# hellobertrand/zxc

Hardware: AMD Instinct MI355X
Metric: seekable decode GB/s (level 3, 64 KiB independent blocks, HBM-resident in/out) (higher is better)
Workload: dtype u8

## Files before the change

### zxc_amd/csrc/zxc_decode_kernel.hip

```cpp
#include "zxc_experiments.h"
#include <hip/hip_runtime.h>
#include <stdint.h>

#include "zxc_kernels.h"
#include "zxc_wave.h"

typedef unsigned __int128 u128;

#include "zxc_lds.h"

#define RING_BYTES 4096u
#define RING_MASK (RING_BYTES - 1u)
#define RING_WORDS (RING_BYTES / 4u)
#define REDIRECT_PASSES 2
#define SPARSE_MAX 8
#define TILE_MAX 3584u
#define LIT_MED 128u
#define MATCH_MED 128u
#define BYTEWISE_MAX 32u

#define E_DST_TOO_SMALL (-2)
#define E_SRC_TOO_SMALL (-3)
#define E_BAD_HEADER (-6)
#define E_BAD_CHECKSUM (-7)
// ... 1133 lines not shown
    }
#ifdef EXP_TIMES
    __builtin_amdgcn_s_waitcnt(0);
    {
        const uint64_t t_end = wall_clock64();
        rc = (int)((((uint32_t)(t_start >> 5) & 0xFFFFu) << 16) | (uint32_t)(((t_end - t_start) >> 5) & 0xFFFFu));
    }
#endif
    if (lane == 0) status[b] = rc == ZXC_DEV_DEFER ? ZXC_DEV_E_INTERNAL : rc;
}

extern "C" __global__ void __launch_bounds__(64, LEAN_WAVES_PER_SIMD)
zxc_decode_blocks_lean_kernel(const uint8_t* __restrict__ comp, const zxc_dev_job_t* __restrict__ jobs, uint32_t n_jobs,
                              uint8_t* __restrict__ out, int32_t* __restrict__ status, uint32_t block_size,
                              const uint32_t* __restrict__ order, uint32_t cap_override, uint32_t trailer_bytes,
                              const zxc_dev_pre_t* __restrict__ pre, const uint8_t* __restrict__ rscratch) {
    __shared__ LeanLds L;
    if (blockIdx.x >= n_jobs) return;
    const uint32_t b = order ? uni(order[blockIdx.x]) : blockIdx.x;
    const uint32_t cls = uni(pre[b].cls);
    if (cls != ZXC_DEV_CLS_LEAN && cls != ZXC_DEV_CLS_LEAN_RLE) return;
    const uint8_t* rle_slot = cls == ZXC_DEV_CLS_LEAN_RLE ? rscratch + 16ull * uni(pre[b].lit_off) : nullptr;
    const int rle_rc = cls == ZXC_DEV_CLS_LEAN_RLE ? (int)(int16_t)uni((uint32_t)(uint16_t)pre[b].rc_lit) : 0;
    lean_one_block<false>(comp, jobs, out, status, block_size, cap_override, trailer_bytes, b, nullptr, nullptr, L, threadIdx.x, rle_slot, rle_rc);
}

extern "C" __global__ void __launch_bounds__(64)
zxc_rle_expand_kernel(const uint8_t* __restrict__ comp, const zxc_dev_job_t* __restrict__ jobs, zxc_dev_pre_t* __restrict__ pre,
                      uint8_t* __restrict__ rscratch, const uint32_t* __restrict__ hdr, const uint32_t* __restrict__ entries_last) {
    const int lane = threadIdx.x;
    const uint32_t n = uni(hdr[0]);
    for (uint32_t i = blockIdx.x; i < n; i += gridDim.x) {
        const uint32_t b = uni(*(entries_last - i));
        const uint8_t* src = comp + jobs[b].comp_off;
        const uint32_t n_lit = uni(ld32(src + 12));
        int rc = 0;
        if (n_lit != 0u) rc = rle_expand(src + 8 + 16, uni(ld32(src + 20)), rscratch + 16ull * uni(pre[b].lit_off) + 16u, n_lit, lane);
        if (lane == 0) pre[b].rc_lit = (int16_t)rc;
    }
}

extern "C" __global__ void __launch_bounds__(64, LEAN_WAVES_PER_SIMD)
zxc_decode_blocks_lean_pre_kernel(const uint8_t* __restrict__ comp, const zxc_dev_job_t* __restrict__ jobs, uint8_t* __restrict__ out,
                                  int32_t* __restrict__ status, uint32_t block_size, uint32_t cap_override, uint32_t trailer_bytes,
                                  const zxc_dev_pre_t* __restrict__ pre, const uint8_t* __restrict__ pscratch,
                                  const uint32_t* __restrict__ hdr, const uint32_t* __restrict__ entries) {
    __shared__ LeanLds L;
    if (blockIdx.x >= uni(hdr[0])) return;
    lean_one_block<true>(comp, jobs, out, status, block_size, cap_override, trailer_bytes, uni(entries[blockIdx.x]), pre, pscratch, L, threadIdx.x, nullptr, 0);
}

extern "C" __global__ void __launch_bounds__(64)
zxc_block_checksum_kernel(const uint8_t* __restrict__ comp, const zxc_dev_job_t* __restrict__ jobs, uint32_t n_jobs,
                          const uint32_t* __restrict__ order, uint8_t* __restrict__ ck_bad) {
    const int lane = threadIdx.x;
    const uint32_t slot = blockIdx.x * 9u + (uint32_t)lane / 7u;
    const bool in = lane < 63 && slot < n_jobs;
    const uint32_t b = in ? (order ? order[slot] : slot) : 0u;
    const uint8_t* src = comp + jobs[b].comp_off;
    const uint32_t src_sz = in ? jobs[b].comp_size : 0u;
    uint32_t comp_sz = 0;
    bool on = false;
    if (src_sz >= 8u) {
        comp_sz = ld32(src + 3);
        on = (uint64_t)8u + comp_sz + 4u <= src_sz;
    }
    const uint32_t h = group_checksum32(src + 8, on ? comp_sz : 0u, lane, on);
    if (on && lane % 7 == 0) ck_bad[b] = h != ld32(src + 8 + comp_sz) ? 1u : 0u;
    else if (in && !on && lane % 7 == 0) ck_bad[b] = 0u;
}
extern "C" __global__ void __launch_bounds__(256)
zxc_checksum_merge_kernel(const uint8_t* __restrict__ ck_bad, int32_t* __restrict__ status, uint32_t n_jobs) {
    const uint32_t i = blockIdx.x * 256u + threadIdx.x;
    if (i < n_jobs && ck_bad[i]) status[i] = E_BAD_CHECKSUM;
}

__device__ __forceinline__ uint32_t order_bucket(const uint8_t* __restrict__ comp, const zxc_dev_job_t& j, uint32_t block_size) {
    uint32_t cost = 0;
    if (j.comp_size >= 8u + 12u) {
        const uint8_t* h = comp + j.comp_off;
        const uint32_t type = ld8(h);
        if (type == 1u || type == 2u) {
            const uint32_t n_seq = ld32(h + 8), n_lit = ld32(h + 12), enc_lit = ld8(h + 16), enc_tok = ld8(h + 17);
            cost = n_seq + (enc_tok == 2u ? n_seq : 0u) + (enc_lit == 1u ? n_lit >> 4 : 0u) + (enc_lit >= 2u ? n_lit >> 2 : 0u);
        }
    }
    const uint64_t q = (uint64_t)cost * 320u / block_size;
    return 63u - (q > 63u ? 63u : (uint32_t)q);
}

extern "C" __global__ void __launch_bounds__(256)
zxc_order_hist_kernel(const uint8_t* __restrict__ comp, const zxc_dev_job_t* __restrict__ jobs, uint32_t n_jobs,
                      uint32_t block_size, uint32_t* __restrict__ hist) {
    __shared__ uint32_t cnt[64];
    if (threadIdx.x < 64u) cnt[threadIdx.x] = 0;
    __syncthreads();
    const uint32_t i = blockIdx.x * 256u + threadIdx.x;
    if (i < n_jobs) atomicAdd(cnt + order_bucket(comp, jobs[i], block_size), 1u);
    __syncthreads();
    if (threadIdx.x < 64u && cnt[threadIdx.x]) atomicAdd(hist + threadIdx.x, cnt[threadIdx.x]);
}

extern "C" __global__ void __launch_bounds__(256)
zxc_order_scatter_kernel(const uint8_t* __restrict__ comp, const zxc_dev_job_t* __restrict__ jobs, uint32_t n_jobs,
                         uint32_t block_size, uint32_t* __restrict__ hist, uint32_t* __restrict__ order,
                         uint32_t* __restrict__ list, uint32_t trailer_bytes, zxc_dev_pre_t* __restrict__ pre,
                         uint32_t* __restrict__ ctl, uint32_t* __restrict__ pre_entries, zxc_dev_sec_t* __restrict__ secs,
                         uint32_t pscratch_cap16, uint32_t cap, uint32_t rscratch_cap16) {
    __shared__ uint32_t cnt[64], base[64];
    __shared__ uint32_t wg_cnt[8], wg_base[8];
    __shared__ uint32_t wg_fit, wg_rle_fit;
    if (threadIdx.x < 64u) cnt[threadIdx.x] = 0;
    if (threadIdx.x < 8u) wg_cnt[threadIdx.x] = 0;
    __syncthreads();
    const uint32_t i = blockIdx.x * 256u + threadIdx.x;
    uint32_t bk = 0, rank = 0;
    if (i < n_jobs) {
        bk = order_bucket(comp, jobs[i], block_size);
        rank = atomicAdd(cnt + bk, 1u);
    }
    __syncthreads();
    if (threadIdx.x < 64u) {
        uint32_t s = 0;
        for (uint32_t k = 0; k < threadIdx.x; k++) s += hist[k];
        base[threadIdx.x] = cnt[threadIdx.x] ? s + atomicAdd(hist + 64u + threadIdx.x, cnt[threadIdx.x]) : 0u;
    }
    __syncthreads();
    if (i < n_jobs) order[base[bk] + rank] = i;
    if (!list) return;
    BlockClass c = {ZXC_DEV_CLS_LEAN, 0, 0, 3, 3, 0, 0, 0, 0, 0, 0};
    uint32_t my_off = 0, my_pre = 0, my_full = 0, my_lit = 0, my_tok = 0;
    if (i < n_jobs) {
        c = classify_block(comp + jobs[i].comp_off, jobs[i].comp_size, trailer_bytes, block_size, cap);
        if (c.cls == ZXC_DEV_CLS_PRE) {
            my_off = atomicAdd(wg_cnt + 0, c.lit16 + c.tok16);
            my_pre = atomicAdd(wg_cnt + 1, 1u);
            if (c.lit_cls < 3u) my_lit = atomicAdd(wg_cnt + 3u + c.lit_cls, 1u);
            if (c.tok_cls < 3u) my_tok = atomicAdd(wg_cnt + 3u + c.tok_cls, 1u);
        } else if (c.cls == ZXC_DEV_CLS_FULL) {
            my_full = atomicAdd(wg_cnt + 2, 1u);
        } else if (c.cls == ZXC_DEV_CLS_LEAN_RLE) {
            my_off = atomicAdd(wg_cnt + 6, c.lit16);
            my_pre = atomicAdd(wg_cnt + 7, 1u);
        }
    }
    __syncthreads();
    if (threadIdx.x == 0) {
        bool rfit = rscratch_cap16 != 0u;
        wg_base[6] = 0;
        if (wg_cnt[7]) {
            atomicAdd(ctl + ZXC_DEV_CTL_RLE_WANTED, wg_cnt[6] + 1u);
            if (wg_cnt[6]) {
                uint32_t old = __hip_atomic_load(ctl + ZXC_DEV_CTL_RLE_CURSOR, __ATOMIC_RELAXED, __HIP_MEMORY_SCOPE_AGENT);
                for (;;) {
                    if (old > rscratch_cap16) { rfit = false; break; }
                    const uint32_t seen = atomicCAS(ctl + ZXC_DEV_CTL_RLE_CURSOR, old, old + wg_cnt[6]);
                    if (seen == old) { rfit = (uint64_t)old + wg_cnt[6] <= rscratch_cap16; break; }
                    old = seen;
                }
                wg_base[6] = old;
            }
            if (!rfit) wg_cnt[2] += wg_cnt[7];
            else wg_base[7] = atomicAdd(ctl + ZXC_DEV_CTL_RLE_LIST, wg_cnt[7]);
        }
        wg_rle_fit = rfit ? 1u : 0u;
        bool fit = true;
        wg_base[0] = 0;
        if (wg_cnt[0]) {
            uint32_t old = __hip_atomic_load(ctl + ZXC_DEV_CTL_CURSOR, __ATOMIC_RELAXED, __HIP_MEMORY_SCOPE_AGENT);
            for (;;) {
                if (old > pscratch_cap16) { fit = false; break; }
                const uint32_t seen = atomicCAS(ctl + ZXC_DEV_CTL_CURSOR, old, old + wg_cnt[0]);
                if (seen == old) { fit = (uint64_t)old + wg_cnt[0] <= pscratch_cap16; break; }
                old = seen;
            }
            wg_base[0] = old;
        }
        wg_fit = fit ? 1u : 0u;
        if (wg_cnt[1]) atomicAdd(ctl + ZXC_DEV_CTL_WANTED, wg_cnt[1]);
        if (fit) {
            wg_base[1] = wg_cnt[1] ? atomicAdd(ctl + ZXC_DEV_CTL_PRE, wg_cnt[1]) : 0u;
            wg_base[2] = wg_cnt[2] ? atomicAdd(list, wg_cnt[2]) : 0u;
            for (uint32_t k = 0; k < 3u; k++) wg_base[3u + k] = wg_cnt[3u + k] ? atomicAdd(ctl + ZXC_DEV_CTL_SEC + 2u * k, wg_cnt[3u + k]) : 0u;
        } else {
            wg_base[2] = atomicAdd(list, wg_cnt[2] + wg_cnt[1]);
        }
    }
    __syncthreads();
    if (i >= n_jobs) return;
    uint32_t cls = c.cls;
    if (cls == ZXC_DEV_CLS_PRE && !wg_fit) {
        cls = ZXC_DEV_CLS_FULL;
        my_full = wg_cnt[2] + my_pre;
    }
    if (cls == ZXC_DEV_CLS_LEAN_RLE) {
        if (wg_rle_fit) {
            pre_entries[n_jobs - 1u - (wg_base[7] + my_pre)] = i;
            pre[i].lit_off = wg_base[6] + my_off;
            pre[i].tok_off = 0;
            pre[i].rc_lit = 0;
            pre[i].rc_tok = 0;
            pre[i].cls = cls;
            return;
        }
        cls = ZXC_DEV_CLS_FULL;
        my_full = wg_cnt[2] - wg_cnt[7] + my_pre;
    }
    const uint32_t off = wg_base[0] + my_off;
    pre[i].lit_off = off;
    pre[i].tok_off = off + c.lit16;
    pre[i].rc_lit = 0;
    pre[i].rc_tok = 0;
    pre[i].cls = cls;
    if (cls == ZXC_DEV_CLS_FULL) {
        list[2u + wg_base[2] + my_full] = base[bk] + rank;
    } else if (cls == ZXC_DEV_CLS_PRE) {
        pre_entries[wg_base[1] + my_pre] = i;
        if (c.lit_cls < 3u) {
            zxc_dev_sec_t& s = secs[(size_t)c.lit_cls * 2u * n_jobs + wg_base[3u + c.lit_cls] + my_lit];
            s.src_off = jobs[i].comp_off + c.lit_at;
            s.psize = c.lit_psize;
            s.n = c.n_lit;
            s.out_off4 = 4u * off + 4u;
            s.rc_slot = 8u * i + 4u;
        }
        if (c.tok_cls < 3u) {
            zxc_dev_sec_t& s = secs[(size_t)c.tok_cls * 2u * n_jobs + wg_base[3u + c.tok_cls] + my_tok];
            s.src_off = jobs[i].comp_off + c.tok_at;
            s.psize = c.tok_psize;
            s.n = c.n_seq;
            s.out_off4 = 4u * (off + c.lit16);
            s.rc_slot = 8u * i + 5u;
        }
    }
}
```

### zxc_amd/csrc/zxc_dev.h

```cpp
#ifndef ZXC_DEV_H
#define ZXC_DEV_H
#include "../../include/zxc_mi355x.h"

#define ZXC_DEV_E_UNSUPPORTED (-101)
#define ZXC_DEV_DEFER (-103)
#define ZXC_DEV_E_INTERNAL (-102)

typedef struct zxc_enc_job {
    uint64_t src_off;
    uint32_t len;
    uint32_t pad;
} zxc_enc_job_t;

#define ZXC_DEV_CLS_LEAN 0u
#define ZXC_DEV_CLS_FULL 1u
#define ZXC_DEV_CLS_PRE 2u
#define ZXC_DEV_CLS_LEAN_RLE 3u
typedef struct {
    uint32_t lit_off;
    uint32_t tok_off;
    int16_t rc_lit, rc_tok;
    uint32_t cls;
} zxc_dev_pre_t;
typedef struct {
    uint64_t src_off;
    uint32_t psize, n;
    uint32_t out_off4;
    uint32_t rc_slot;
    uint32_t pad[2];
} zxc_dev_sec_t;
#define ZXC_DEV_TRAILER_ELSEWHERE 0x80000000u
#define ZXC_DEV_CTL_WORDS 32u
#define ZXC_DEV_CTL_PRE 0u
#define ZXC_DEV_CTL_CURSOR 2u
#define ZXC_DEV_CTL_WANTED 3u
#define ZXC_DEV_CTL_SEC 4u
#define ZXC_DEV_CTL_RLE_CURSOR 10u
#define ZXC_DEV_CTL_RLE_WANTED 11u
#define ZXC_DEV_CTL_RLE_LIST 12u

#define ZXC_DEV_SLOT_REGION(bs) ((bs) + 64u)
#define ZXC_DEV_SLOT_STRIDE(bs) ((2u * ZXC_DEV_SLOT_REGION(bs) + (bs) / 5u + 16u + 64u + 255u) & ~255u)

typedef struct { size_t list, order, ctl, pre_ent, secs, pre, ck_bad, words; } zxc_dev_ord_layout_t;
static inline zxc_dev_ord_layout_t zxc_dev_ord_layout(uint32_t n_jobs) {
    const size_t n = n_jobs, ctl = 130u + 2u * n, pre_ent = ctl + ZXC_DEV_CTL_WORDS, secs = (pre_ent + n + 7u) & ~(size_t)7u;
    const zxc_dev_ord_layout_t l = {128u, 130u + n, ctl, pre_ent, secs, secs + 48u * n, secs + 52u * n, secs + 52u * n + (n + 3u) / 4u};
    return l;
}

enum { ZXC_DEV_PLAN_FULL, ZXC_DEV_PLAN_DICT, ZXC_DEV_PLAN_TWO_PASS, ZXC_DEV_PLAN_TWO_PASS_PRE };
#define ZXC_DEV_DBG_NO_TWO_PASS 0x40000000u
#define ZXC_DEV_DBG_NO_ORDER 0x80000000u
typedef struct {
    uint32_t kind, ordered, ck_apart, trailer_bytes;
    uint64_t pscratch_bytes, rscratch_bytes;
} zxc_dev_plan_t;
typedef struct {
    uint32_t dict, cap_override, n_jobs, max_slots, debug, verify_trailer, block_size;
    uint32_t slot, helpers, hint, hint0, hint1;
    uint32_t ck_inline, no_rle_scratch, rle_lean_max_jobs, no_pre;
    uint32_t order_failed, pscratch_failed, rscratch_failed;
} zxc_dev_plan_in_t;

static inline zxc_dev_plan_t zxc_dev_plan_choose(const zxc_dev_plan_in_t* in) {
    const uint64_t gib = (uint64_t)1 << 30, n = in->n_jobs, bs = in->block_size;
    const int two_pass = !in->dict && !in->cap_override && !(in->debug & ZXC_DEV_DBG_NO_TWO_PASS);
    const int wants_order = two_pass || (in->n_jobs > in->max_slots && !(in->debug & ZXC_DEV_DBG_NO_ORDER));
    zxc_dev_plan_t p = {in->dict ? ZXC_DEV_PLAN_DICT : ZXC_DEV_PLAN_FULL, wants_order && in->slot && !in->order_failed, 0u,
                        in->verify_trailer ? 4u : 0u, 0u, 0u};
    if (!two_pass || !p.ordered || !in->helpers) return p;
    p.kind = (!in->hint || in->hint0 != 0u) && !in->no_pre && !in->pscratch_failed ? ZXC_DEV_PLAN_TWO_PASS_PRE : ZXC_DEV_PLAN_TWO_PASS;
    if (p.kind == ZXC_DEV_PLAN_TWO_PASS_PRE) p.pscratch_bytes = n * (bs + bs / 5u + 256u) < gib ? n * (bs + bs / 5u + 256u) : gib;
    if (in->hint && n < in->rle_lean_max_jobs && in->hint1 && !in->no_rle_scratch && !in->rscratch_failed) {
        const uint64_t need = ((uint64_t)in->hint1 * 16u * 5u / 4u + 65536u) & ~(uint64_t)4095u, most = n * (bs + 96u) < gib ? n * (bs + 96u) : gib;
        p.rscratch_bytes = need < most ? need : most;
    }
    p.ck_apart = p.kind == ZXC_DEV_PLAN_TWO_PASS && in->verify_trailer && !in->ck_inline;
    if (p.ck_apart) p.trailer_bytes |= ZXC_DEV_TRAILER_ELSEWHERE;
    return p;
}
#endif
```

### zxc_amd/csrc/zxc_experiments.h

```cpp
#ifndef ZXC_EXPERIMENTS_H
#define ZXC_EXPERIMENTS_H
#ifndef ZXC_EXPERIMENT
#if defined(ASM_MARKERS) || defined(EXP_ENC_CLOCKS) || defined(EXP_NO_PRE) || defined(EXP_PHASES) || defined(EXP_PIV_PROF) || defined(EXP_TIMES)
#error "an experiment switch is defined without -DZXC_EXPERIMENT: this is not the product configuration (zxc_experiments.h)"
#endif
#endif
#endif
```

### zxc_amd/csrc/zxc_hip_shim.hip

```cpp
#include "zxc_experiments.h"
#include <hip/hip_runtime.h>
#include <pthread.h>
#include <stdint.h>
#include <stdlib.h>

#include "../../include/zxc_error.h"
#include "zxc_encode_levels.h"
#include "zxc_kernels.h"

#ifdef EXP_ENC_CLOCKS
extern "C" __attribute__((visibility("default"))) int zxc_mi355x_exp_enc_clocks(unsigned long long* out8) {
    unsigned long long* d = NULL;
    if (hipMalloc((void**)&d, 64) != hipSuccess) return -1;
    hipLaunchKernelGGL(zxc_enc_clk_read_kernel, dim3(1), dim3(64), 0, 0, d);
    const hipError_t e = hipMemcpy(out8, d, 64, hipMemcpyDeviceToHost);
    (void)hipFree(d);
    return e == hipSuccess ? 0 : -1;
}
#endif

#define ZXC_MAX_DEVICES 16
#define ZXC_RLE_LEAN_MAX_JOBS 16384u
#define ZXC_ORDER_STREAMS 16
#define ZXC_POOLS 10
struct Pool { uint8_t* scratch; uint32_t* busy; uint32_t n_slots; uint32_t stride; };
struct Ord {
    void* stream; int used; uint32_t* buf; size_t buf_cap; hipStream_t aux, aux2; hipEvent_t fork, join, join2, small_done;
    uint32_t* hint; uint8_t* pscratch; size_t pscratch_cap; uint8_t* rscratch; size_t rscratch_cap;
};
static struct {
    Pool pool[ZXC_POOLS];
    int cus, wg_per_cu;
    Ord ord[ZXC_ORDER_STREAMS];
} g_dev[ZXC_MAX_DEVICES];
static pthread_mutex_t g_lock = PTHREAD_MUTEX_INITIALIZER;

#ifdef ZXC_EXPERIMENT
static uint32_t g_debug_flags = 0;
#else
#define g_debug_flags 0u
#endif

static int current_device(void) {
    int d = -1;
    if (hipGetDevice(&d) != hipSuccess || d < 0 || d >= ZXC_MAX_DEVICES) return -1;
    return d;
}

extern "C" {

#ifdef ZXC_EXPERIMENT
__attribute__((visibility("default"))) void zxc_mi355x__set_debug(uint32_t flags) { g_debug_flags = flags; }
#endif

int zxc_mi355x_device_count(void) {
    int n = 0;
    if (hipGetDeviceCount(&n) != hipSuccess) return 0;
    return n;
}

int zxc_mi355x_set_device(int device) {
    return hipSetDevice(device) == hipSuccess ? ZXC_OK : ZXC_ERROR_GPU_UNAVAILABLE;
}

int zxc_mi355x_get_device(void) {
    int d = -1;
    return hipGetDevice(&d) == hipSuccess ? d : ZXC_ERROR_GPU_UNAVAILABLE;
}

void* zxc_mi355x_malloc(size_t bytes) {
    void* p = NULL;
    if (hipMalloc(&p, bytes ? bytes : 16) != hipSuccess) return NULL;
    return p;
}

void zxc_mi355x_free(void* d_ptr) {
    if (d_ptr) (void)hipFree(d_ptr);
}

int zxc_mi355x_memcpy_h2d(void* d_dst, const void* h_src, size_t bytes) {
    if (bytes == 0) return ZXC_OK;
    return hipMemcpy(d_dst, h_src, bytes, hipMemcpyHostToDevice) == hipSuccess ? ZXC_OK : ZXC_ERROR_GPU_UNAVAILABLE;
}

int zxc_mi355x_memcpy_d2h(void* h_dst, const void* d_src, size_t bytes) {
// ... 33 lines not shown
    *ev_out = (void*)e;
    return ZXC_OK;
}
void zxc_hip_event_destroy(void* ev) { if (ev) (void)hipEventDestroy((hipEvent_t)ev); }
int zxc_hip_event_record(void* ev, void* stream) {
    return hipEventRecord((hipEvent_t)ev, (hipStream_t)stream) == hipSuccess ? ZXC_OK : ZXC_ERROR_GPU_UNAVAILABLE;
}
int zxc_hip_event_synchronize(void* ev) {
    return hipEventSynchronize((hipEvent_t)ev) == hipSuccess ? ZXC_OK : ZXC_ERROR_GPU_UNAVAILABLE;
}
void* zxc_hip_host_alloc(size_t bytes) {
    void* p = NULL;
    if (hipHostMalloc(&p, bytes ? bytes : 16, hipHostMallocDefault) != hipSuccess) return NULL;
    return p;
}
void zxc_hip_host_free(void* p) { if (p) (void)hipHostFree(p); }

extern "C" void zxc_host_release_arenas(void);
void zxc_mi355x_release_cached(void) {
    zxc_host_release_arenas();
    const int dev = current_device();
    if (dev < 0) return;
    (void)hipDeviceSynchronize();
    pthread_mutex_lock(&g_lock);
    for (int i = 0; i < ZXC_POOLS; i++) {
        auto& p = g_dev[dev].pool[i];
        if (p.scratch) (void)hipFree(p.scratch);
        if (p.busy) (void)hipFree(p.busy);
        p.scratch = NULL; p.busy = NULL; p.n_slots = 0; p.stride = 0;
    }
    for (int i = 0; i < ZXC_ORDER_STREAMS; i++) {
        auto& o = g_dev[dev].ord[i];
        if (o.buf) (void)hipFree(o.buf);
        if (o.pscratch) (void)hipFree(o.pscratch);
        if (o.rscratch) (void)hipFree(o.rscratch);
        o.buf = NULL; o.buf_cap = 0;
        o.pscratch = NULL; o.pscratch_cap = 0;
        o.rscratch = NULL; o.rscratch_cap = 0;
    }
    pthread_mutex_unlock(&g_lock);
}

int zxc_mi355x_synchronize(void* stream) {
    return hipStreamSynchronize((hipStream_t)stream) == hipSuccess ? ZXC_OK : ZXC_ERROR_GPU_UNAVAILABLE;
}

static int setup_pool(int dev, uint32_t block_size, Pool** pool_out, uint32_t* max_slots) {
    auto& d = g_dev[dev];
    if (d.cus == 0 && (hipDeviceGetAttribute(&d.cus, hipDeviceAttributeMultiprocessorCount, dev) != hipSuccess || d.cus <= 0)) d.cus = 256;
    if (d.wg_per_cu == 0 && (hipOccupancyMaxActiveBlocksPerMultiprocessor(&d.wg_per_cu, zxc_decode_blocks_kernel, 64, 0) != hipSuccess ||
                             d.wg_per_cu <= 0 || d.wg_per_cu > 32))
        d.wg_per_cu = 32;
    *max_slots = (uint32_t)d.cus * (uint32_t)d.wg_per_cu;
    Pool& pool = *(*pool_out = &d.pool[__builtin_ctz(block_size) - 12]);
    if (pool.scratch) return ZXC_OK;
    const uint32_t stride = ZXC_DEV_SLOT_STRIDE(block_size);
    uint32_t n = (uint32_t)(((size_t)1 << 30) / stride);
    if (n > *max_slots) n = *max_slots;
    if (n < 64u) n = 64u;
    uint8_t* sc = NULL;
    uint32_t* busy = NULL;
    if (hipMalloc((void**)&sc, (size_t)n * stride) != hipSuccess) return ZXC_ERROR_MEMORY;
    if (hipMalloc((void**)&busy, (size_t)n * 4u) != hipSuccess) { (void)hipFree(sc); return ZXC_ERROR_MEMORY; }
    if (hipMemset(busy, 0, (size_t)n * 4u) != hipSuccess || hipDeviceSynchronize() != hipSuccess) {
        (void)hipFree(sc), (void)hipFree(busy);
        return ZXC_ERROR_GPU_UNAVAILABLE;
    }
    pool = Pool{sc, busy, n, stride};
    return ZXC_OK;
}

static Ord* claim_slot(int dev, void* stream) {
    Ord* ord = g_dev[dev].ord;
    for (int i = 0; i < ZXC_ORDER_STREAMS; i++)
        if (ord[i].used && ord[i].stream == stream) return &ord[i];
    for (int i = 0; i < ZXC_ORDER_STREAMS; i++)
        if (!ord[i].used) {
            ord[i].used = 1, ord[i].stream = stream;
            if (ord[i].hint) { ord[i].hint[0] = 0xFFFFFFFFu; ord[i].hint[1] = 0u; }
            return &ord[i];
        }
    return NULL;
}

static void make_helpers(Ord& o) {
    if (o.aux) return;
    if (hipStreamCreateWithFlags(&o.aux, hipStreamNonBlocking) != hipSuccess) { o.aux = NULL; return; }
    const unsigned f = hipEventDisableTiming;
    if (hipStreamCreateWithFlags(&o.aux2, hipStreamNonBlocking) != hipSuccess) { (void)hipStreamDestroy(o.aux); o.aux = NULL; return; }
    if (hipEventCreateWithFlags(&o.fork, f) != hipSuccess || hipEventCreateWithFlags(&o.join, f) != hipSuccess ||
        hipEventCreateWithFlags(&o.join2, f) != hipSuccess || hipEventCreateWithFlags(&o.small_done, f) != hipSuccess) {
        (void)hipStreamDestroy(o.aux), (void)hipStreamDestroy(o.aux2);
        o.aux = NULL;
    } else if (!o.hint) {
        if (hipHostMalloc((void**)&o.hint, 64, hipHostMallocDefault) == hipSuccess) { o.hint[0] = 0xFFFFFFFFu; o.hint[1] = 0u; }
        else o.hint = NULL;
    }
}

static bool grow(void** p, size_t* cap, size_t bytes) {
    if (*cap >= bytes) return true;
    if (*p) (void)hipFree(*p);
    *cap = 0;
    if (hipMalloc(p, bytes) != hipSuccess) { *p = NULL; return false; }
    *cap = bytes;
    return true;
}

struct Launch {
    const uint8_t* comp; const zxc_dev_job_t* jobs; uint32_t n; uint8_t* out; int32_t* status; uint32_t bs, cap_override;
    zxc_dev_plan_t plan; hipStream_t s0; const Pool* pool; uint32_t max_slots, cus; Ord* o;
    uint32_t *order, *list, *ctl, *pre_entries; zxc_dev_sec_t* secs; zxc_dev_pre_t* pre;
    uint8_t *ck_bad, *pscratch, *rscratch; uint32_t pscratch_cap16, rscratch_cap16;
};

static void order_pass(const Launch& L) {
    const uint32_t g = (L.n + 255u) / 256u;
    hipLaunchKernelGGL(zxc_order_hist_kernel, dim3(g), dim3(256), 0, L.s0, L.comp, L.jobs, L.n, L.bs, L.o->buf);
    hipLaunchKernelGGL(zxc_order_scatter_kernel, dim3(g), dim3(256), 0, L.s0, L.comp, L.jobs, L.n, L.bs, L.o->buf, L.order, L.list,
                       L.plan.trailer_bytes & ~ZXC_DEV_TRAILER_ELSEWHERE, L.pre, L.ctl, L.pre_entries, L.secs, L.pscratch_cap16,
                       L.cap_override ? L.cap_override : L.bs + 2112u, L.rscratch_cap16);
    if (L.ctl && L.o->hint) {
        (void)hipMemcpyAsync(L.o->hint, L.ctl + ZXC_DEV_CTL_WANTED, 4, hipMemcpyDeviceToHost, L.s0);
        (void)hipMemcpyAsync(L.o->hint + 1, L.ctl + ZXC_DEV_CTL_RLE_WANTED, 4, hipMemcpyDeviceToHost, L.s0);
    }
}

static void launch_full(const Launch& L, hipStream_t st, uint32_t grid) {
    hipLaunchKernelGGL(zxc_decode_blocks_kernel, dim3(grid), dim3(64), 0, st, L.comp, L.jobs, L.n, L.out, L.status, L.bs, L.plan.trailer_bytes,
                       L.pool->scratch, L.pool->stride, g_debug_flags, L.pool->busy, L.pool->n_slots, L.order, L.cap_override, L.list);
}

static void launch_rle(const Launch& L, hipStream_t st) {
    if (!L.rscratch_cap16) return;
    hipLaunchKernelGGL(zxc_rle_expand_kernel, dim3(L.n < 8u * L.cus ? L.n : 8u * L.cus), dim3(64), 0, st, L.comp, L.jobs, L.pre,
                       L.rscratch, L.ctl + ZXC_DEV_CTL_RLE_LIST, L.pre_entries + L.n - 1u);
}

static bool fork_to(Ord& o, hipStream_t h) { return hipStreamWaitEvent(h, o.fork, 0) == hipSuccess; }
static int fail(Ord& o) { (void)hipStreamSynchronize(o.aux), (void)hipStreamSynchronize(o.aux2); return ZXC_ERROR_GPU_UNAVAILABLE; }
static int join(Ord& o, hipStream_t s0, bool aux, bool aux2) {
    if ((aux && (hipEventRecord(o.join, o.aux) != hipSuccess || hipStreamWaitEvent(s0, o.join, 0) != hipSuccess)) ||
        (aux2 && (hipEventRecord(o.join2, o.aux2) != hipSuccess || hipStreamWaitEvent(s0, o.join2, 0) != hipSuccess)))
        return fail(o);
    return ZXC_OK;
}

static int enqueue_two_pass(const Launch& L) {
    Ord& o = *L.o; const hipStream_t s0 = L.s0;
    const bool aux = hipEventRecord(o.fork, s0) == hipSuccess && fork_to(o, o.aux);
    launch_full(L, aux ? o.aux : s0, L.n < L.max_slots ? L.n : L.max_slots);
    const bool aux2 = L.plan.ck_apart && aux && fork_to(o, o.aux2);
    if (L.plan.ck_apart)
        hipLaunchKernelGGL(zxc_block_checksum_kernel, dim3((L.n + 8u) / 9u), dim3(64), 0, aux2 ? o.aux2 : s0, L.comp, L.jobs, L.n, L.order, L.ck_bad);
    launch_rle(L, s0);
    hipLaunchKernelGGL(zxc_decode_blocks_lean_kernel, dim3(L.n), dim3(64), 0, s0, L.comp, L.jobs, L.n, L.out, L.status, L.bs, L.order,
                       L.cap_override, L.plan.trailer_bytes, L.pre, L.rscratch);
    if (const int rc = join(o, s0, aux, aux2)) return rc;
    if (L.plan.ck_apart)
        hipLaunchKernelGGL(zxc_checksum_merge_kernel, dim3((L.n + 255u) / 256u), dim3(256), 0, s0, L.ck_bad, L.status, L.n);
    return ZXC_OK;
}

static int enqueue_two_pass_pre(const Launch& L) {
    Ord& o = *L.o;
    const bool forked = hipEventRecord(o.fork, L.s0) == hipSuccess && fork_to(o, o.aux) && fork_to(o, o.aux2);
    const hipStream_t s0 = L.s0, s1 = forked ? o.aux : s0, s2 = forked ? o.aux2 : s0;
    uint32_t* sec_hdr = L.ctl + ZXC_DEV_CTL_SEC;
    auto grid = [&](uint32_t per_cu) { const uint32_t g = per_cu * L.cus; return dim3(2u * L.n < g ? 2u * L.n : g); };
    launch_rle(L, s1);
    hipLaunchKernelGGL(zxc_decode_blocks_lean_kernel, dim3(L.n), dim3(64), 0, s1, L.comp, L.jobs, L.n, L.out, L.status, L.bs, L.order,
                       L.cap_override, L.plan.trailer_bytes, L.pre, L.rscratch);
    hipLaunchKernelGGL(zxc_pivco_sections_small_kernel, grid(10), dim3(PDIR_SMALL_THREADS), 0, s2, L.comp, L.secs, sec_hdr, L.pre, L.pscratch);
    if (forked && hipEventRecord(o.small_done, s2) != hipSuccess) return fail(o);
    launch_full(L, s2, L.n < L.max_slots ? L.n : L.max_slots);
    hipLaunchKernelGGL(zxc_pivco_sections_medium_kernel, grid(3), dim3(PDIR_MEDIUM_THREADS), 0, s0, L.comp, L.secs + 2u * (size_t)L.n, sec_hdr + 2, L.pre, L.pscratch);
    hipLaunchKernelGGL(zxc_pivco_sections_large_kernel, grid(2), dim3(PDIR_LARGE_THREADS), 0, s0, L.comp, L.secs + 4u * (size_t)L.n, sec_hdr + 4, L.pre, L.pscratch);
    if (forked && hipStreamWaitEvent(s0, o.small_done, 0) != hipSuccess) return fail(o);
    hipLaunchKernelGGL(zxc_decode_blocks_lean_pre_kernel, dim3(L.n), dim3(64), 0, s0, L.comp, L.jobs, L.out, L.status, L.bs,
                       L.cap_override, L.plan.trailer_bytes, L.pre, L.pscratch, L.ctl + ZXC_DEV_CTL_PRE, L.pre_entries);
    return join(o, s0, forked, forked);
}

static int decode_launch(const void* d_comp, const zxc_dev_job_t* d_jobs, uint32_t n_jobs, void* d_out,
                         int32_t* d_status, uint32_t block_size, int verify_trailer, void* stream, const void* d_dict,
                         uint32_t dict_size, const void* d_dict_huf, uint32_t cap_override = 0) {
    if (n_jobs == 0) return ZXC_OK;
    if (!d_comp || !d_jobs || !d_out || !d_status) return ZXC_ERROR_NULL_INPUT;
    if (block_size < (1u << 12) || block_size > (1u << 21) || (block_size & (block_size - 1u))) return ZXC_ERROR_BAD_BLOCK_SIZE;
    const int dev = current_device();
    if (dev < 0) return ZXC_ERROR_GPU_UNAVAILABLE;
    zxc_dev_plan_in_t in = {(uint32_t)(d_dict || d_dict_huf), cap_override, n_jobs, 0u, g_debug_flags, (uint32_t)(verify_trailer != 0), block_size};
    in.rle_lean_max_jobs = ZXC_RLE_LEAN_MAX_JOBS;
    in.ck_inline = getenv("ZXC_MI355X_CK_INLINE") != NULL, in.no_rle_scratch = getenv("ZXC_MI355X_NO_RLE_SCRATCH") != NULL;
#ifdef EXP_NO_PRE
    in.no_pre = 1;
#endif
    struct Unlock { ~Unlock() { pthread_mutex_unlock(&g_lock); } } unlock_on_return;
    pthread_mutex_lock(&g_lock);
    Pool* pool;
    if (const int rc = setup_pool(dev, block_size, &pool, &in.max_slots)) return rc;
    in.slot = in.helpers = 1;
    const zxc_dev_plan_t could = zxc_dev_plan_choose(&in);
    Ord* o = could.ordered ? claim_slot(dev, stream) : NULL;
    if (o && could.kind >= ZXC_DEV_PLAN_TWO_PASS) make_helpers(*o);
    in.slot = o != NULL; in.helpers = o && o->aux; in.hint = o && o->hint;
    if (in.hint) { in.hint0 = *(volatile uint32_t*)o->hint; in.hint1 = *(volatile uint32_t*)(o->hint + 1); }
    zxc_dev_plan_t plan = zxc_dev_plan_choose(&in);
    const hipStream_t s0 = (hipStream_t)stream; const zxc_dev_ord_layout_t at = zxc_dev_ord_layout(n_jobs);
    if (plan.ordered) in.order_failed = !grow((void**)&o->buf, &o->buf_cap, at.words * 4u);
    if (plan.pscratch_bytes) in.pscratch_failed = !grow((void**)&o->pscratch, &o->pscratch_cap, plan.pscratch_bytes);
    if (plan.rscratch_bytes) in.rscratch_failed = !grow((void**)&o->rscratch, &o->rscratch_cap, plan.rscratch_bytes);
    if (plan.ordered && !in.order_failed)
        in.order_failed = hipMemsetAsync(o->buf, 0, 130u * 4u, s0) != hipSuccess ||
                          hipMemsetAsync(o->buf + at.ctl, 0, ZXC_DEV_CTL_WORDS * 4u, s0) != hipSuccess;
    plan = zxc_dev_plan_choose(&in);
    Launch L = {(const uint8_t*)d_comp, d_jobs, n_jobs, (uint8_t*)d_out, d_status, block_size, cap_override, plan, s0, pool,
                in.max_slots, (uint32_t)g_dev[dev].cus, o};
    if (plan.ordered) L.order = o->buf + at.order;
    if (plan.kind >= ZXC_DEV_PLAN_TWO_PASS) {
        L.list = o->buf + at.list; L.ctl = o->buf + at.ctl; L.pre_entries = o->buf + at.pre_ent;
        L.secs = (zxc_dev_sec_t*)(o->buf + at.secs); L.pre = (zxc_dev_pre_t*)(o->buf + at.pre); L.ck_bad = (uint8_t*)(o->buf + at.ck_bad);
        if (plan.pscratch_bytes) { L.pscratch = o->pscratch; L.pscratch_cap16 = (uint32_t)(o->pscratch_cap >> 4); }
        if (plan.rscratch_bytes) { L.rscratch = o->rscratch; L.rscratch_cap16 = (uint32_t)(o->rscratch_cap >> 4); }
    }
    if (plan.ordered) order_pass(L);
    if (plan.kind == ZXC_DEV_PLAN_TWO_PASS || plan.kind == ZXC_DEV_PLAN_TWO_PASS_PRE) {
        if (const int rc = plan.kind == ZXC_DEV_PLAN_TWO_PASS ? enqueue_two_pass(L) : enqueue_two_pass_pre(L)) return rc;
    } else if (plan.kind == ZXC_DEV_PLAN_DICT)
        hipLaunchKernelGGL(zxc_decode_blocks_dict_kernel, dim3(n_jobs), dim3(64), 0, s0, L.comp, d_jobs, n_jobs, L.out, d_status, block_size,
                           plan.trailer_bytes, pool->scratch, pool->stride, g_debug_flags, pool->busy, pool->n_slots, L.order, cap_override,
                           (const uint8_t*)d_dict, dict_size, (const uint8_t*)d_dict_huf);
    else
        launch_full(L, s0, n_jobs);
    return hipGetLastError() == hipSuccess ? ZXC_OK : ZXC_ERROR_GPU_UNAVAILABLE;
}

int zxc_mi355x_decode_blocks_device(const void* d_comp, const zxc_dev_job_t* d_jobs, uint32_t n_jobs, void* d_out,
                                    int32_t* d_status, uint32_t block_size, int verify_trailer, void* stream) {
    return decode_launch(d_comp, d_jobs, n_jobs, d_out, d_status, block_size, verify_trailer, stream, NULL, 0, NULL);
}

int zxc_mi355x_decode_blocks_dict_device(const void* d_comp, const zxc_dev_job_t* d_jobs, uint32_t n_jobs, void* d_out,
                                         int32_t* d_status, uint32_t block_size, int verify_trailer, const void* d_dict,
                                         uint32_t dict_size, const void* d_dict_huf, void* stream) {
    if (dict_size > 65535u || (dict_size && !d_dict)) return ZXC_ERROR_DICT_TOO_LARGE;
    return decode_launch(d_comp, d_jobs, n_jobs, d_out, d_status, block_size, verify_trailer, stream, d_dict, dict_size,
                         d_dict_huf);
}

int zxc_hip_decode_blocks(const void* d_comp, const zxc_dev_job_t* d_jobs, uint32_t n_jobs, void* d_out, int32_t* d_status,
                          uint32_t block_size, int verify_trailer, const void* d_dict, uint32_t dict_size,
                          const void* d_dict_huf, uint32_t cap_override, void* stream) {
    if (dict_size > 65535u || (dict_size && !d_dict)) return ZXC_ERROR_DICT_TOO_LARGE;
    return decode_launch(d_comp, d_jobs, n_jobs, d_out, d_status, block_size, verify_trailer, stream, d_dict, dict_size,
                         d_dict_huf, cap_override);
}
int zxc_hip_current_device(void) { return current_device(); }

uint32_t zxc_mi355x_encode_slot_stride(uint32_t block_size) { return 2u * block_size + 512u; }

static int encode_launch(const void* d_src, uint64_t src_size, uint32_t block_size, int level, int with_checksum,
                         const void* d_dict, uint32_t dict_size, void* d_work, void* d_slots, uint32_t* d_sizes, void* stream) {
    if (src_size == 0) return ZXC_OK;
    if (!d_src || !d_slots || !d_sizes || (dict_size && (!d_dict || !d_work))) return ZXC_ERROR_NULL_INPUT;
    if (block_size < (1u << 12) || block_size > (1u << 21) || (block_size & (block_size - 1u))) return ZXC_ERROR_BAD_BLOCK_SIZE;
    if (dict_size > 65535u) return ZXC_ERROR_DICT_TOO_LARGE;
    if (current_device() < 0) return ZXC_ERROR_GPU_UNAVAILABLE;
    const uint64_t nb64 = (src_size + block_size - 1u) / block_size;
    if (nb64 > 0x7FFFFFFFull) return ZXC_ERROR_BAD_BLOCK_SIZE;
    const uint32_t nb = (uint32_t)nb64;
// ... 85 lines not shown
```

### zxc_amd/csrc/zxc_kernels.h

```cpp
#ifndef ZXC_KERNELS_H
#define ZXC_KERNELS_H
#include <hip/hip_runtime.h>
#include <stdint.h>

#include "zxc_container.h"
#include "zxc_dev.h"

#define PDIR_SMALL_THREADS 128
#define PDIR_MEDIUM_THREADS 256
#define PDIR_LARGE_THREADS 512

extern "C" __global__ void zxc_decode_blocks_kernel(const uint8_t* comp, const zxc_dev_job_t* jobs, uint32_t n_jobs,
                                                    uint8_t* out, int32_t* status, uint32_t block_size,
                                                    uint32_t trailer_bytes, uint8_t* scratch, uint32_t scratch_stride, uint32_t dbg,
                                                    uint32_t* slot_busy, uint32_t n_slots, const uint32_t* order,
                                                    uint32_t cap_override, uint32_t* list);
extern "C" __global__ void zxc_decode_blocks_dict_kernel(const uint8_t* comp, const zxc_dev_job_t* jobs, uint32_t n_jobs,
                                                         uint8_t* out, int32_t* status, uint32_t block_size,
                                                         uint32_t trailer_bytes, uint8_t* scratch, uint32_t scratch_stride,
                                                         uint32_t dbg, uint32_t* slot_busy, uint32_t n_slots,
                                                         const uint32_t* order, uint32_t cap_override, const uint8_t* dict,
                                                         uint32_t dict_size, const uint8_t* dict_huf);
extern "C" __global__ void zxc_decode_blocks_lean_kernel(const uint8_t* comp, const zxc_dev_job_t* jobs, uint32_t n_jobs,
                                                         uint8_t* out, int32_t* status, uint32_t block_size,
                                                         const uint32_t* order, uint32_t cap_override, uint32_t trailer_bytes,
                                                         const zxc_dev_pre_t* pre, const uint8_t* rscratch);
extern "C" __global__ void zxc_decode_blocks_lean_pre_kernel(const uint8_t* comp, const zxc_dev_job_t* jobs, uint8_t* out, int32_t* status,
                                                             uint32_t block_size, uint32_t cap_override, uint32_t trailer_bytes,
                                                             const zxc_dev_pre_t* pre, const uint8_t* pscratch, const uint32_t* hdr,
                                                             const uint32_t* entries);
extern "C" __global__ void zxc_rle_expand_kernel(const uint8_t* comp, const zxc_dev_job_t* jobs, zxc_dev_pre_t* pre, uint8_t* rscratch,
                                                 const uint32_t* hdr, const uint32_t* entries_last);
extern "C" __global__ void zxc_order_hist_kernel(const uint8_t* comp, const zxc_dev_job_t* jobs, uint32_t n_jobs,
                                                 uint32_t block_size, uint32_t* hist);
extern "C" __global__ void zxc_order_scatter_kernel(const uint8_t* comp, const zxc_dev_job_t* jobs, uint32_t n_jobs,
                                                    uint32_t block_size, uint32_t* hist, uint32_t* order, uint32_t* list, uint32_t trailer_bytes,
                                                    zxc_dev_pre_t* pre, uint32_t* ctl, uint32_t* pre_entries, zxc_dev_sec_t* secs,
                                                    uint32_t pscratch_cap16, uint32_t cap, uint32_t rscratch_cap16);
#define ZXC_SECTIONS_KERNEL(name)                                                                                              \
    extern "C" __global__ void name(const uint8_t* comp, const zxc_dev_sec_t* secs, uint32_t* hdr, zxc_dev_pre_t* pre, uint8_t* pscratch)
ZXC_SECTIONS_KERNEL(zxc_pivco_sections_small_kernel);
ZXC_SECTIONS_KERNEL(zxc_pivco_sections_medium_kernel);
ZXC_SECTIONS_KERNEL(zxc_pivco_sections_large_kernel);
#undef ZXC_SECTIONS_KERNEL
extern "C" __global__ void zxc_block_checksum_kernel(const uint8_t* comp, const zxc_dev_job_t* jobs, uint32_t n_jobs, const uint32_t* order, uint8_t* ck_bad);
extern "C" __global__ void zxc_checksum_merge_kernel(const uint8_t* ck_bad, int32_t* status, uint32_t n_jobs);

#define ZXC_ENCODE_DECL(name)                                                                                          \
    extern "C" __global__ void name(const uint8_t* src, uint64_t src_size, uint32_t block_size, uint8_t* slots,        \
                                    uint32_t slot_stride, uint32_t* sizes, uint32_t n_blocks, uint32_t with_checksum,  \
                                    uint32_t depth, uint32_t sufficient, uint32_t lazy, uint32_t dict_size,        \
                                    uint8_t* huf_scratch, uint32_t huf)
ZXC_ENCODE_DECL(zxc_encode_blocks_kernel_l1);
ZXC_ENCODE_DECL(zxc_encode_blocks_kernel_l2);
ZXC_ENCODE_DECL(zxc_encode_blocks_kernel_l3);
ZXC_ENCODE_DECL(zxc_encode_blocks_kernel_l4);
ZXC_ENCODE_DECL(zxc_encode_blocks_kernel_l57);
ZXC_ENCODE_DECL(zxc_encode_blocks_kernel_l67);
#undef ZXC_ENCODE_DECL
#define ZXC_ENCODE_JOBS_DECL(name)                                                                                     \
    extern "C" __global__ void name(const uint8_t* src, const zxc_enc_job_t* jobs, uint32_t block_size, uint8_t* slots, \
                                    uint32_t slot_stride, uint32_t* sizes, uint32_t n_jobs, uint32_t with_checksum,    \
                                    uint32_t depth, uint32_t sufficient, uint32_t lazy, uint32_t dict_size,            \
                                    uint8_t* huf_scratch, uint32_t huf)
ZXC_ENCODE_JOBS_DECL(zxc_encode_jobs_kernel_l1);
ZXC_ENCODE_JOBS_DECL(zxc_encode_jobs_kernel_l2);
ZXC_ENCODE_JOBS_DECL(zxc_encode_jobs_kernel_l3);
ZXC_ENCODE_JOBS_DECL(zxc_encode_jobs_kernel_l4);
ZXC_ENCODE_JOBS_DECL(zxc_encode_jobs_kernel_l57);
ZXC_ENCODE_JOBS_DECL(zxc_encode_jobs_kernel_l67);
#undef ZXC_ENCODE_JOBS_DECL
extern "C" __global__ void zxc_prepend_dict_kernel(const uint8_t* src, uint64_t src_size, uint32_t block_size, const uint8_t* dict,
                                                   uint32_t dict_size, uint8_t* work, uint32_t n_blocks);
extern "C" __global__ void zxc_encode_job_images_kernel(const uint8_t* src, zxc_enc_job_t* jobs, uint32_t n, uint32_t block_size,
                                                        const uint8_t* dict, uint32_t dict_size, uint8_t* work);
extern "C" __global__ void zxc_block_offsets_kernel(uint32_t* sizes, uint64_t* offsets, uint32_t n_blocks, uint32_t max_size);
extern "C" __global__ void zxc_gather_blocks_kernel(const uint8_t* slots, uint32_t slot_stride, const uint32_t* sizes,
                                                    const uint64_t* offsets, uint8_t* out, uint32_t n_blocks);

extern "C" __global__ void zxc_unframe_head_kernel(const uint8_t* src, uint64_t src_size, uint64_t dst_capacity, uint32_t block_size,
                                                   uint32_t want_verify, uint32_t n_jobs, zc_ctl_t* ctl, const uint32_t* dict_id);
extern "C" __global__ void zxc_unframe_tiles_kernel(const uint8_t* src, const zc_ctl_t* ctl, uint64_t* tile_sum, uint32_t* tile_bad);
extern "C" __global__ void zxc_unframe_scan_kernel(uint64_t* tile_sum, const uint32_t* tile_bad, uint32_t n_tiles, zc_ctl_t* ctl);
extern "C" __global__ void zxc_unframe_scatter_kernel(const uint8_t* src, const zc_ctl_t* ctl, const uint64_t* tile_off, uint32_t block_size,
                                                      uint32_t k_direct, uint32_t n_jobs, zxc_dev_job_t* jobs, uint32_t* tile_hash,
                                                      uint32_t* tile_bad);
extern "C" __global__ void zxc_unframe_walk_kernel(const uint8_t* src, uint64_t src_size, uint32_t block_size, uint32_t k_direct,
                                                   uint32_t n_jobs, const uint32_t* tile_hash, const uint32_t* tile_bad, zxc_dev_job_t* jobs,
                                                   zc_ctl_t* ctl);
extern "C" __global__ void zxc_unframe_events_kernel(const int32_t* status, uint32_t block_size, uint32_t n_jobs, uint64_t dst_capacity,
                                                     zc_ctl_t* ctl);
extern "C" __global__ void zxc_unframe_result_kernel(const zc_ctl_t* ctl, const int32_t* status, uint32_t block_size, uint32_t n_jobs,
                                                     int64_t* result);
#ifdef EXP_ENC_CLOCKS
extern "C" __global__ void zxc_enc_clk_read_kernel(unsigned long long* out);
#endif
#endif
```

Baseline: 1014.

## Interleave sorted block order across columns to balance lean decode waves

The order scatter kernel now permutes each block's sorted position through a row/column transpose (61 rows), leaving only the last 2×resident-slots entries in sorted order. Heavy and light blocks are therefore spread across concurrently resident workgroups rather than grouped together, while the tail keeps the longest-first ordering. The checksum kernel and full-class list use the same mapped positions so all consumers agree. The host queries lean-kernel occupancy to size the tail. This costs a few integer divisions per job and may reduce locality among neighbouring blocks.

```diff
diff --git a/zxc_amd/csrc/zxc_decode_kernel.hip b/zxc_amd/csrc/zxc_decode_kernel.hip
--- a/zxc_amd/csrc/zxc_decode_kernel.hip
+++ b/zxc_amd/csrc/zxc_decode_kernel.hip
@@ -1209,11 +1209,11 @@
 
 extern "C" __global__ void __launch_bounds__(64)
 zxc_block_checksum_kernel(const uint8_t* __restrict__ comp, const zxc_dev_job_t* __restrict__ jobs, uint32_t n_jobs,
-                          const uint32_t* __restrict__ order, uint8_t* __restrict__ ck_bad) {
+                          const uint32_t* __restrict__ order, uint8_t* __restrict__ ck_bad, uint32_t mix_slots) {
     const int lane = threadIdx.x;
     const uint32_t slot = blockIdx.x * 9u + (uint32_t)lane / 7u;
     const bool in = lane < 63 && slot < n_jobs;
-    const uint32_t b = in ? (order ? order[slot] : slot) : 0u;
+    const uint32_t b = in ? (order ? order[zxc_dev_order_mix(slot, n_jobs, mix_slots)] : slot) : 0u;
     const uint8_t* src = comp + jobs[b].comp_off;
     const uint32_t src_sz = in ? jobs[b].comp_size : 0u;
     uint32_t comp_sz = 0;
@@ -1263,7 +1263,7 @@
                          uint32_t block_size, uint32_t* __restrict__ hist, uint32_t* __restrict__ order,
                          uint32_t* __restrict__ list, uint32_t trailer_bytes, zxc_dev_pre_t* __restrict__ pre,
                          uint32_t* __restrict__ ctl, uint32_t* __restrict__ pre_entries, zxc_dev_sec_t* __restrict__ secs,
-                         uint32_t pscratch_cap16, uint32_t cap, uint32_t rscratch_cap16) {
+                         uint32_t pscratch_cap16, uint32_t cap, uint32_t rscratch_cap16, uint32_t mix_slots) {
     __shared__ uint32_t cnt[64], base[64];
     __shared__ uint32_t wg_cnt[8], wg_base[8];
     __shared__ uint32_t wg_fit, wg_rle_fit;
@@ -1283,7 +1283,11 @@
         base[threadIdx.x] = cnt[threadIdx.x] ? s + atomicAdd(hist + 64u + threadIdx.x, cnt[threadIdx.x]) : 0u;
     }
     __syncthreads();
-    if (i < n_jobs) order[base[bk] + rank] = i;
+    uint32_t pos = i < n_jobs ? zxc_dev_order_mix(base[bk] + rank, n_jobs, mix_slots) : 0u;
+#ifdef ZXC_EXPERIMENT
+    if (mix_slots == 0xFFFFFFFFu) pos = i;
+#endif
+    if (i < n_jobs) order[pos] = i;
     if (!list) return;
     BlockClass c = {ZXC_DEV_CLS_LEAN, 0, 0, 3, 3, 0, 0, 0, 0, 0, 0};
     uint32_t my_off = 0, my_pre = 0, my_full = 0, my_lit = 0, my_tok = 0;
@@ -1370,7 +1374,7 @@
     pre[i].rc_tok = 0;
     pre[i].cls = cls;
     if (cls == ZXC_DEV_CLS_FULL) {
-        list[2u + wg_base[2] + my_full] = base[bk] + rank;
+        list[2u + wg_base[2] + my_full] = pos;
     } else if (cls == ZXC_DEV_CLS_PRE) {
         pre_entries[wg_base[1] + my_pre] = i;
         if (c.lit_cls < 3u) {
diff --git a/zxc_amd/csrc/zxc_dev.h b/zxc_amd/csrc/zxc_dev.h
--- a/zxc_amd/csrc/zxc_dev.h
+++ b/zxc_amd/csrc/zxc_dev.h
@@ -49,6 +49,26 @@
     return l;
 }
 
+#ifndef EXP_ORDER_MIX_ROWS
+#define ZXC_DEV_ORDER_MIX_ROWS 61u
+#else
+#define ZXC_DEV_ORDER_MIX_ROWS EXP_ORDER_MIX_ROWS
+#endif
+#ifdef __HIPCC__
+__host__ __device__
+#endif
+static inline uint32_t zxc_dev_order_mix(uint32_t pos, uint32_t n, uint32_t slots) {
+    const uint64_t tail = 2ull * slots;
+    if (slots == 0u || n <= tail) return pos;
+    const uint32_t head = n - (uint32_t)tail, rows = ZXC_DEV_ORDER_MIX_ROWS;
+    if (pos >= head) return pos;
+    const uint32_t c_long = (head + rows - 1u) / rows, q = head - rows * (c_long - 1u);
+    uint32_t r, c;
+    if (pos < q * c_long) { r = pos / c_long; c = pos % c_long; }
+    else { const uint32_t p = pos - q * c_long; r = q + p / (c_long - 1u); c = p % (c_long - 1u); }
+    return c * rows + r;
+}
+
 enum { ZXC_DEV_PLAN_FULL, ZXC_DEV_PLAN_DICT, ZXC_DEV_PLAN_TWO_PASS, ZXC_DEV_PLAN_TWO_PASS_PRE };
 #define ZXC_DEV_DBG_NO_TWO_PASS 0x40000000u
 #define ZXC_DEV_DBG_NO_ORDER 0x80000000u
diff --git a/zxc_amd/csrc/zxc_experiments.h b/zxc_amd/csrc/zxc_experiments.h
--- a/zxc_amd/csrc/zxc_experiments.h
+++ b/zxc_amd/csrc/zxc_experiments.h
@@ -1,7 +1,8 @@
 #ifndef ZXC_EXPERIMENTS_H
 #define ZXC_EXPERIMENTS_H
 #ifndef ZXC_EXPERIMENT
-#if defined(ASM_MARKERS) || defined(EXP_ENC_CLOCKS) || defined(EXP_NO_PRE) || defined(EXP_PHASES) || defined(EXP_PIV_PROF) || defined(EXP_TIMES)
+#if defined(ASM_MARKERS) || defined(EXP_ENC_CLOCKS) || defined(EXP_NO_PRE) || defined(EXP_PHASES) || defined(EXP_PIV_PROF) || defined(EXP_TIMES) || \
+    defined(EXP_ORDER_MIX_ROWS)
 #error "an experiment switch is defined without -DZXC_EXPERIMENT: this is not the product configuration (zxc_experiments.h)"
 #endif
 #endif
diff --git a/zxc_amd/csrc/zxc_hip_shim.hip b/zxc_amd/csrc/zxc_hip_shim.hip
--- a/zxc_amd/csrc/zxc_hip_shim.hip
+++ b/zxc_amd/csrc/zxc_hip_shim.hip
@@ -30,7 +30,7 @@
 };
 static struct {
     Pool pool[ZXC_POOLS];
-    int cus, wg_per_cu;
+    int cus, wg_per_cu, lean_wg_per_cu;
     Ord ord[ZXC_ORDER_STREAMS];
 } g_dev[ZXC_MAX_DEVICES];
 static pthread_mutex_t g_lock = PTHREAD_MUTEX_INITIALIZER;
@@ -170,6 +170,9 @@
                              d.wg_per_cu <= 0 || d.wg_per_cu > 32))
         d.wg_per_cu = 32;
     *max_slots = (uint32_t)d.cus * (uint32_t)d.wg_per_cu;
+    if (d.lean_wg_per_cu == 0 && (hipOccupancyMaxActiveBlocksPerMultiprocessor(&d.lean_wg_per_cu, zxc_decode_blocks_lean_kernel, 64, 0) != hipSuccess ||
+                                  d.lean_wg_per_cu <= 0 || d.lean_wg_per_cu > 32))
+        d.lean_wg_per_cu = 24;
     Pool& pool = *(*pool_out = &d.pool[__builtin_ctz(block_size) - 12]);
     if (pool.scratch) return ZXC_OK;
     const uint32_t stride = ZXC_DEV_SLOT_STRIDE(block_size);
@@ -227,7 +230,7 @@
 
 struct Launch {
     const uint8_t* comp; const zxc_dev_job_t* jobs; uint32_t n; uint8_t* out; int32_t* status; uint32_t bs, cap_override;
-    zxc_dev_plan_t plan; hipStream_t s0; const Pool* pool; uint32_t max_slots, cus; Ord* o;
+    zxc_dev_plan_t plan; hipStream_t s0; const Pool* pool; uint32_t max_slots, cus, mix_slots; Ord* o;
     uint32_t *order, *list, *ctl, *pre_entries; zxc_dev_sec_t* secs; zxc_dev_pre_t* pre;
     uint8_t *ck_bad, *pscratch, *rscratch; uint32_t pscratch_cap16, rscratch_cap16;
 };
@@ -237,7 +240,7 @@
     hipLaunchKernelGGL(zxc_order_hist_kernel, dim3(g), dim3(256), 0, L.s0, L.comp, L.jobs, L.n, L.bs, L.o->buf);
     hipLaunchKernelGGL(zxc_order_scatter_kernel, dim3(g), dim3(256), 0, L.s0, L.comp, L.jobs, L.n, L.bs, L.o->buf, L.order, L.list,
                        L.plan.trailer_bytes & ~ZXC_DEV_TRAILER_ELSEWHERE, L.pre, L.ctl, L.pre_entries, L.secs, L.pscratch_cap16,
-                       L.cap_override ? L.cap_override : L.bs + 2112u, L.rscratch_cap16);
+                       L.cap_override ? L.cap_override : L.bs + 2112u, L.rscratch_cap16, L.mix_slots);
     if (L.ctl && L.o->hint) {
         (void)hipMemcpyAsync(L.o->hint, L.ctl + ZXC_DEV_CTL_WANTED, 4, hipMemcpyDeviceToHost, L.s0);
         (void)hipMemcpyAsync(L.o->hint + 1, L.ctl + ZXC_DEV_CTL_RLE_WANTED, 4, hipMemcpyDeviceToHost, L.s0);
@@ -270,7 +273,7 @@
     launch_full(L, aux ? o.aux : s0, L.n < L.max_slots ? L.n : L.max_slots);
     const bool aux2 = L.plan.ck_apart && aux && fork_to(o, o.aux2);
     if (L.plan.ck_apart)
-        hipLaunchKernelGGL(zxc_block_checksum_kernel, dim3((L.n + 8u) / 9u), dim3(64), 0, aux2 ? o.aux2 : s0, L.comp, L.jobs, L.n, L.order, L.ck_bad);
+        hipLaunchKernelGGL(zxc_block_checksum_kernel, dim3((L.n + 8u) / 9u), dim3(64), 0, aux2 ? o.aux2 : s0, L.comp, L.jobs, L.n, L.order, L.ck_bad, L.mix_slots);
     launch_rle(L, s0);
     hipLaunchKernelGGL(zxc_decode_blocks_lean_kernel, dim3(L.n), dim3(64), 0, s0, L.comp, L.jobs, L.n, L.out, L.status, L.bs, L.order,
                        L.cap_override, L.plan.trailer_bytes, L.pre, L.rscratch);
@@ -334,7 +337,10 @@
                           hipMemsetAsync(o->buf + at.ctl, 0, ZXC_DEV_CTL_WORDS * 4u, s0) != hipSuccess;
     plan = zxc_dev_plan_choose(&in);
     Launch L = {(const uint8_t*)d_comp, d_jobs, n_jobs, (uint8_t*)d_out, d_status, block_size, cap_override, plan, s0, pool,
-                in.max_slots, (uint32_t)g_dev[dev].cus, o};
+                in.max_slots, (uint32_t)g_dev[dev].cus, (uint32_t)g_dev[dev].cus * (uint32_t)g_dev[dev].lean_wg_per_cu, o};
+#ifdef ZXC_EXPERIMENT
+    if (const char* e = getenv("ZXC_EXP_ORDER_SLOTS")) L.mix_slots = (uint32_t)strtoul(e, NULL, 0);
+#endif
     if (plan.ordered) L.order = o->buf + at.order;
     if (plan.kind >= ZXC_DEV_PLAN_TWO_PASS) {
         L.list = o->buf + at.list; L.ctl = o->buf + at.ctl; L.pre_entries = o->buf + at.pre_ent;
diff --git a/zxc_amd/csrc/zxc_kernels.h b/zxc_amd/csrc/zxc_kernels.h
--- a/zxc_amd/csrc/zxc_kernels.h
+++ b/zxc_amd/csrc/zxc_kernels.h
@@ -36,14 +36,15 @@
 extern "C" __global__ void zxc_order_scatter_kernel(const uint8_t* comp, const zxc_dev_job_t* jobs, uint32_t n_jobs,
                                                     uint32_t block_size, uint32_t* hist, uint32_t* order, uint32_t* list, uint32_t trailer_bytes,
                                                     zxc_dev_pre_t* pre, uint32_t* ctl, uint32_t* pre_entries, zxc_dev_sec_t* secs,
-                                                    uint32_t pscratch_cap16, uint32_t cap, uint32_t rscratch_cap16);
+                                                    uint32_t pscratch_cap16, uint32_t cap, uint32_t rscratch_cap16, uint32_t mix_slots = 0u);
 #define ZXC_SECTIONS_KERNEL(name)                                                                                              \
     extern "C" __global__ void name(const uint8_t* comp, const zxc_dev_sec_t* secs, uint32_t* hdr, zxc_dev_pre_t* pre, uint8_t* pscratch)
 ZXC_SECTIONS_KERNEL(zxc_pivco_sections_small_kernel);
 ZXC_SECTIONS_KERNEL(zxc_pivco_sections_medium_kernel);
 ZXC_SECTIONS_KERNEL(zxc_pivco_sections_large_kernel);
 #undef ZXC_SECTIONS_KERNEL
-extern "C" __global__ void zxc_block_checksum_kernel(const uint8_t* comp, const zxc_dev_job_t* jobs, uint32_t n_jobs, const uint32_t* order, uint8_t* ck_bad);
+extern "C" __global__ void zxc_block_checksum_kernel(const uint8_t* comp, const zxc_dev_job_t* jobs, uint32_t n_jobs, const uint32_t* order, uint8_t* ck_bad,
+                                                     uint32_t mix_slots = 0u);
 extern "C" __global__ void zxc_checksum_merge_kernel(const uint8_t* ck_bad, int32_t* status, uint32_t n_jobs);
 
 #define ZXC_ENCODE_DECL(name)                                                                                          \
```

After: 1036 (median of 6 runs). 1.02x the previous value.
